# fgiral000/gencast-flax-nnx

Hardware: AMD Instinct MI355X
Metric: denoiser-calls/sec (higher is better)
Workload: dtype f16x3 (every product = 3 fp16 MFMAs on hi/lo-split f32 operands: 22-bit products, f32 accumulate; f32 storage); 1 GPU; nano-GenCast DPM-Solver++2S 20-step sample, 2.5deg grid (73x144), 1 ensemble member per GPU, batch 1; dead_call_skipped=True, grid_nodes=10512, mesh_nodes=2562, latent=256, layers=16, heads=4, ffw_hidden=2048, c_in=262, c_out=82, k_hop=8, parallelism=ensemble-dp1, broadcast=none, rccl_ranks=0, precision=f16x3, library_built_from_this_tree=True, launcher=single

## Files before the change

gencast-flax-nnx_amd/csrc/gc_api.hip:

```cpp
#include <dlfcn.h>

#include "gc_handle.h"

using namespace gci;

namespace {

void protect_pending_noise(gc_handle* h) {
  if (h->guard_pending && h->d_noise == h->last_noise) std::swap(h->d_noise, h->d_noise_alt);
}

int check_ready(gc_handle* h) {
  if (!h) return GC_ERR_INVALID_ARGUMENT;
  if (!h->finalized) return fail(h, GC_ERR_STATE, "gc_finalize has not been called");
  return GC_OK;
}

struct Rccl {
  void* lib = nullptr;
  ncclResult_t (*GetUniqueId)(ncclUniqueId*) = nullptr;
  ncclResult_t (*CommInitRank)(ncclComm_t*, int, ncclUniqueId, int) = nullptr;
  ncclResult_t (*CommDestroy)(ncclComm_t) = nullptr;
  ncclResult_t (*CommCount)(const ncclComm_t, int*) = nullptr;
  ncclResult_t (*CommUserRank)(const ncclComm_t, int*) = nullptr;
// ... 97 lines not shown
  if (hipGetDeviceCount(&n) != hipSuccess) return 0;
  return n;
}

int gc_device_pci_bus_id(int32_t device_id, char* out, int64_t cap) {
  if (!out || cap < 16 || device_id < 0 || device_id >= gc_device_count()) return GC_ERR_INVALID_ARGUMENT;
  out[0] = 0;
  return hipDeviceGetPCIBusId(out, (int)cap, device_id) == hipSuccess ? GC_OK : GC_ERR_HIP;
}

const char* gc_last_error(const gc_handle* h) { return h ? h->err.c_str() : g_create_error.c_str(); }

static void read_switches(gc_handle* h) {
  auto is = [](const char* name, const char* value) { const char* v = std::getenv(name); return v && std::string(v) == value; };
  auto off = [](const char* name) { const char* v = std::getenv(name); return v && *v && std::atoi(v) == 0; };
  auto on = [](const char* name) { const char* v = std::getenv(name); return v && *v == '1'; };
  h->f16x3 = !is("GC_PRECISION", "f32");
  h->use_graphs = !is("GC_TUNE_GRAPH", "0");
  h->m2g_fuse_sum = !off("GC_TUNE_M2G_FUSE_SUM");
  h->embed_cache = !off("GC_TUNE_EMBED_CACHE");
  h->attn_items = !off("GC_TUNE_ATTN_ITEMS");
  h->mlp_pair = !off("GC_TUNE_MLP_PAIR");
  h->edge_terms = !off("GC_TUNE_EDGE_TERMS");
  h->a16 = !off("GC_TUNE_A16");
  h->graph_serialize = on("GC_TUNE_GRAPH_SERIALIZE");
  h->graph_verbose = on("GC_TUNE_GRAPH_VERBOSE");
  h->poison = on("GC_DEBUG_POISON");
}

int gc_create(const gc_config* cfg, int device_id, gc_handle** out) {
  return guarded(nullptr, [&]() -> int {
  if (!cfg || !out) { g_create_error = "null argument"; return GC_ERR_INVALID_ARGUMENT; }
  *out = nullptr;
  const gc_config& c = *cfg;
  auto bad = [&](const char* m) { g_create_error = m; return GC_ERR_INVALID_ARGUMENT; };
  if (c.latent_size <= 0 || c.d_model <= 0 || c.num_heads <= 0 || c.ffw_hidden <= 0 ||
      c.num_layers < 0 || c.c_in <= 0 || c.c_out <= 0 || c.batch <= 0)
    return bad("all dimensions must be positive");
  if (c.c_out > c.c_in) return bad("c_out cannot exceed c_in (noisy targets are part of the forcings)");
  if (c.latent_size != c.d_model) return bad("latent_size must equal d_model");
  if (c.d_model % c.num_heads) return bad("num_heads has to divide d_model exactly");
  if (c.noise_num_frequencies <= 0 || c.noise_num_frequencies > 128 || c.noise_hidden <= 0 ||
      c.noise_hidden > 128 || !(c.noise_base_period > 0))
    return bad("noise encoder sizes out of range");
  auto unsup = [&](const char* m) { g_create_error = m; return GC_ERR_UNSUPPORTED; };
  if (c.latent_size != 128 && c.latent_size != 256 && c.latent_size != 512)
// ... 675 lines not shown
    double n = 1;
    for (auto d : kv.second) n *= (double)d;
    params += n;
  }
  *bytes = 4.0 * (params + G * (c.c_in + c.c_out) + 2 * G * L + NL * M * D * 10);
  *flops = f;
  return GC_OK;
  });
}

int gc_get_counter(gc_handle* h, const char* name, int64_t* value) {
  return guarded(h, [&]() -> int {
  if (!h) return GC_ERR_INVALID_ARGUMENT;
  if (!name || !value) return fail(h, GC_ERR_INVALID_ARGUMENT, "null argument");
  const std::string n(name);
  if (n == "range_fallbacks") *value = h->range_fallbacks;
  else if (n == "static_embedding_fallbacks") *value = h->static_embedding_fallbacks;
  else if (n == "launches_per_call") *value = h->launches_last_call;
  else if (n == "weights_f16_unsafe") *value = h->weights_f16_unsafe ? 1 : 0;
  else if (n == "fp16_storage") *value = h->last_route.st16 ? 1 : 0;
  else if (n == "split_edge") *value = h->split_edge ? 1 : 0;
  else if (n == "attention_items") *value = h->last_route.att_items;
  else if (n == "m2g_fused_sum") *value = h->last_route.m2g_fused ? 1 : 0;
  else if (n == "embed_cache") *value = h->embed_cache_samples;
  else if (n == "edge_term_samples") *value = h->edge_term_samples;
  else if (n == "edge_term_cache_bytes") *value = h->terms.ready ? h->terms.bytes : 0;
  else if (n == "graph_replays") *value = h->graph_replays;
  else if (n == "graph_captures") *value = h->graph_captures;
  else if (n == "loss_evaluations") *value = h->loss_evaluations;
  else if (n == "loss_device_us") *value = h->loss_device_us;
  else if (const int64_t* v = meter_counter(h, n)) *value = *v;
  else if (n == "ens_window_pushes") *value = h->win_pushes;
  else if (n == "ens_window_ring_bytes") {
    const size_t L = h->win_allocs.key[0], M = h->win_allocs.key[1];
    *value = (int64_t)(L * (((M + 1) * h->hg.G * h->cfg.batch * h->cfg.c_out + 3) / 4 * 4) * sizeof(float));
  }
  else if (n == "ens_map_bytes") *value = h->map_set ? h->map_bytes : 0;
  else if (n == "poison_allocs") *value = h->poison_allocs;
  else if (n == "poison_bytes") *value = h->poison_bytes;
  else if (n == "noise_stream") *value = (int64_t)h->nz_stream;
  else if (n == "device_allocations") {
    *value = 0;
    for (const BufferGroup* g : h->groups) *value += (int64_t)g->ptrs.size();
  }
  else return fail(h, GC_ERR_INVALID_ARGUMENT, "unknown counter: " + n);
  return GC_OK;
// ... 499 lines not shown
```

gencast-flax-nnx_amd/csrc/gc_forward.hip:

```cpp
#include "gc_handle.h"

namespace gci {

template <class To, class From>
static const To& a16_view(const From& v) {
  static_assert(sizeof(To) == sizeof(From), "argument struct mismatch between the two kernel builds");
  return reinterpret_cast<const To&>(v);
}

Route make_route(const gc_handle* h) {
  const int D = h->cfg.d_model, F = h->cfg.ffw_hidden;
  Route r;
  r.f16 = h->f16x3 && !h->weights_f16_unsafe && !h->in_fallback;
  r.x32 = !r.f16 && h->f32_ws;
  const bool streams = r.f16 || r.x32;
  r.ffw_slabs = streams ? h->ffw_fused_slabs : 0;
  r.st16 = h->feat16 && h->a16 && r.f16 && D % 128 == 0 && D <= 512 &&
           (h->ffw_fused_slabs > 0 || (F % 128 == 0 && (F / h->ffw2_splits) % 128 == 0));
  r.v2 = r.f16 && r.ws(3 * D, D, 1);
  r.att_items = (h->att_n_items > 0 && r.ws(3 * D, D, 1) && h->attn_splits == 1 && D <= 512) ? h->att_n_items : 0;
  r.fuse_row = streams && D % 128 == 0 && D <= 512;
  r.node_ws = r.f16;
  r.split_edge = h->split_edge;
  r.try_pair = h->mlp_pair && h->hidden_layers == 1;
  r.m2g_fused = h->m2g_fuse_sum && h->hg.m2g_tri && h->hidden_layers == 1 && streams;
  r.embed_cache = h->embed_cache_live && h->embed_cache_ready && !h->feat16 && h->hidden_layers == 1 && streams;
  r.edge_terms = h->embed_cache_live && h->terms.ready && edge_terms_possible(h) && r.f16;
  return r;
}

bool edge_terms_possible(const gc_handle* h) {
  return h->edge_terms && h->f16x3 && !h->weights_f16_unsafe && !h->in_fallback && !h->feat16 && h->hidden_layers == 1 &&
         h->cfg.latent_size == 256 && h->cfg.batch == 1 && h->hg.m2g_tri;
}

static gc::Segment seg(const float* ptr, const int* index, const float* affine, int width, int ld, int bcast) {
  gc::Segment s;
  s.ptr = ptr; s.index = index; s.affine = affine; s.width = width; s.ld = ld; s.bcast = bcast;
  return s;
}

struct MlpCall {
  gc::Segment seg[3] = {};
  gc::AddTerm add[3] = {};
  int nseg = 0, nadd = 0, rows = 0, B = 1, ldo = 0;
  bool ln = true, cond = true;
  const float* residual = nullptr;
// ... 33 lines not shown
  a.cond_stride = h->cond_total;
  a.residual = c.residual; a.out = c.out; a.ldo = c.ldo;
  a.round16 = h->feat16 ? 1 : 0;
  a.round_out = (h->feat16 && c.round_out) ? 1 : 0;
  a.a16 = r.st16 ? 1 : 0;
  a.seg0_f32 = c.seg0_f32 ? 1 : 0;
  a.out_f32 = c.out_f32 ? 1 : 0;
  a.tri = c.tri ? 1 : 0;
  if (c.tri && !gc::mlp_runs_weight_streaming(a))
    return fail(h, GC_ERR_INTERNAL, "the triple-sum epilogue exists in the weight-streaming MLP kernel only");
  return GC_OK;
}

static int enqueue_mlp(gc_handle* h, const gc::MlpArgs& a) {
  return launch(h, gc::KC_MLP, [&] {
    return a.a16 ? gc_a16::launch_mlp(h->stream, a16_view<gc_a16::MlpArgs>(a)) : gc::launch_mlp(h->stream, a);
  });
}
static int enqueue_mlp_pair(gc_handle* h, const gc::MlpArgs& a, const gc::MlpArgs& b) {
  return launch(h, gc::KC_MLP, [&] {
    return a.a16 ? gc_a16::launch_mlp_pair(h->stream, a16_view<gc_a16::MlpArgs>(a), a16_view<gc_a16::MlpArgs>(b))
                 : gc::launch_mlp_pair(h->stream, a, b);
  });
}
static int enqueue_gemm_ws(gc_handle* h, int cls, const gc::GemmArgs& ga, int mt, int splits, int epi) {
  return launch(h, cls, [&] {
    return ga.a16 ? gc_a16::launch_gemm_ws(h->stream, cls, a16_view<gc_a16::GemmArgs>(ga), mt, splits, epi)
                  : gc::launch_gemm_ws(h->stream, cls, ga, mt, splits, epi);
  });
}
static int enqueue_gemm_rowop(gc_handle* h, int cls, const gc::GemmArgs& ga, const gc::RowFuse& rf) {
  return launch(h, cls, [&] {
    return ga.a16 ? gc_a16::launch_gemm_rowop(h->stream, cls, a16_view<gc_a16::GemmArgs>(ga), a16_view<gc_a16::RowFuse>(rf))
                  : gc::launch_gemm_rowop(h->stream, cls, ga, rf);
  });
}
static int enqueue_ffw_fused(gc_handle* h, const gc::FfwArgs& fa) {
  return launch(h, gc::KC_GEMM_FFW1, [&] {
    return fa.a16 ? gc_a16::launch_ffw_fused(h->stream, a16_view<gc_a16::FfwArgs>(fa)) : gc::launch_ffw_fused(h->stream, fa);
  });
}

static int run_mlp_one(gc_handle* h, const DevMlp& w, const MlpCall& c) {
  gc::MlpArgs a{};
  if (int rc = build_mlp_args(h, w, c, &a)) return rc;
  return enqueue_mlp(h, a);
// ... 138 lines not shown
static int mesh_gemm(gc_handle* h, int cls, const float* a, int lda, const Weight& w, int n, int k, int splits,
                     const float* bias, int act, float* out, int ldo, int epi, bool att_merge = false) {
  const Route& r = h->route;
  const bool ws = r.ws(n, k, splits);
  gc::GemmArgs ga = mesh_gemm_args(h, a, lda, ws);
  ga.wt = pick(w, r, ws ? Form::Streaming : Form::Staged); ga.ldw = k; ga.n = n; ga.k_slice = k / splits;
  ga.bias = bias; ga.act = act; ga.out = out; ga.ldo = ldo;
  if (att_merge) merge_attention_partials(h, &ga);
  if (ws) return enqueue_gemm_ws(h, cls, ga, att_merge ? 1 : pick_ws_mt(ga.rows, n, splits), splits, epi);
  return launch(h, cls, [&] { return gc::launch_gemm(h->stream, cls, ga, splits, epi, r.f16); });
}

int forward(gc_handle* h, float sigma_scalar, const float* cond_ready) {
  const gc_config& c = h->cfg;
  const gc::HostGraph& g = h->hg;
  const int B = c.batch, L = c.latent_size, D = c.d_model, F = c.ffw_hidden;
  hipStream_t s = h->stream;
  int rc;
  const float* cond = cond_ready ? cond_ready : h->d_cond;
  h->cond_cur = cond;
  const int cs = h->cond_total;
  const int64_t launches0 = h->launch_count;
  const Route& r = h->route = h->last_route = make_route(h);

  if (!cond_ready && (rc = launch(h, gc::KC_COND, [&] {
         return gc::launch_cond(s, sigma_scalar < 0 ? h->d_sigma : nullptr, sigma_scalar, B, h->d_nw0t,
                                h->d_nb0, h->d_nw1t, h->d_nb1, c.noise_num_frequencies, c.noise_hidden,
                                c.noise_base_period, h->d_wc_all, h->d_bc_all, cs, h->d_condvec,
                                h->d_cond);
       })))
    return rc;

  {
    MlpCall embed = r.embed_cache ? mlp_call({seg(h->d_xn, nullptr, nullptr, h->nwp, h->nwp, 0)}, g.G * B, B, h->d_g0, L)
                                  : mlp_call({seg(h->d_xp, nullptr, nullptr, h->kp, h->kp, 0)}, g.G * B, B, h->d_g0, L);
    embed.seg0_f32 = true;
    if (r.embed_cache) embed.add_terms({{h->d_pstat, nullptr}});
    if ((rc = run_mlp(h, r.embed_cache ? h->g2m_embed_grid_n : h->g2m_embed_grid, embed))) return rc;
  }
  const size_t ML = (size_t)g.M * L;
  if (r.edge_terms && (h->term_slot < 0 || !h->terms.ready))
    return fail(h, GC_ERR_INTERNAL, "edge terms: the forward has no slot of the cache");
  const float* const m0 = r.edge_terms ? h->terms.m0 + h->term_slot * ML : h->d_m0;
  h->m0_cur = m0;
  if (!r.edge_terms && (rc = launch(h, gc::KC_PACK, [&] {
         return gc::launch_affine_rows(s, h->d_m0_hat, cond + h->g2m_embed_mesh.cond_off, cs, g.M, B, L,
// ... 78 lines not shown
    }
    if (stop_here(i, 2)) return GC_OK;
    if (r.ffw_slabs > 0) {
      gc::FfwArgs fa{h->d_h, MB, (int)D, (int)F, pick(ly.w1, r, Form::Streaming), ly.b1, pick(ly.w2, r, Form::Streaming),
                     h->d_part, h->feat16 ? 1 : 0, r.st16 ? 1 : 0};
      fa.f32w = r.x32 ? 1 : 0;
      if ((rc = enqueue_ffw_fused(h, fa))) return rc;
    } else {
      if ((rc = mesh_gemm(h, gc::KC_GEMM_FFW1, h->d_h, D, ly.w1, F, D, 1, ly.b1, 1, h->d_u, F, 0))) return rc;
      if ((rc = mesh_gemm(h, gc::KC_GEMM_FFW2, h->d_u, F, ly.w2, D, F, h->ffw2_splits, nullptr, 0, h->d_part, D, 1))) return rc;
    }
    pend_bias = ly.b2;
    pend_slabs = r.ffw_slabs > 0 ? r.ffw_slabs : h->ffw2_splits;
  }
  if ((rc = rowop(pend_bias, pend_slabs, h->cond_final, h->d_m2))) return rc;

  if ((r.split_edge || r.edge_terms) && (rc = edge_node_products(h, h->m2g_edge, h->d_m2, g.M * B, h->d_pm, h->d_g1, g.G * B, h->d_pg)))
    return rc;
  if ((rc = run_m2g_edge(h, cond, r.m2g_fused))) return rc;
  if (!r.m2g_fused && (rc = launch(h, gc::KC_SEGSUM, [&] {
         return gc::launch_segsum(s, h->d_f1, h->d_m2g_ptr, h->d_m2g_eid, g.G, g.E2, B, L, h->d_agg2, h->feat16, r.st16);
       })))
    return rc;
  if ((rc = run_mlp(h, h->m2g_grid, mlp_call({seg(h->d_g1, nullptr, nullptr, L, L, 0), seg(h->d_agg2, nullptr, nullptr, L, L, 0)},
                                             g.G * B, B, h->d_g2, L, h->d_g1))))
    return rc;
  MlpCall dec = mlp_call({seg(h->d_g2, nullptr, nullptr, L, L, 0)}, g.G * B, B, h->d_y, c.c_out);
  dec.ln = dec.cond = false; dec.out_f32 = true;
  if ((rc = run_mlp(h, h->m2g_dec, dec))) return rc;
  h->launches_last_call = h->launch_count - launches0;
  return GC_OK;
}

int compute_static_embeddings(gc_handle* h) {
  const gc::HostGraph& hg = h->hg;
  const int L = h->cfg.latent_size;
  const struct { const DevMlp& w; const float* in; int items; float* out; } embeds[] = {
      {h->g2m_embed_mesh, h->d_mesh_struct16, hg.M, h->d_m0_hat},
      {h->g2m_embed_edge, h->d_e1_struct16, hg.E1, h->d_e0_hat},
      {h->m2g_embed_edge, h->d_e2_struct16, hg.E2, h->d_f0_hat}};
  if (int rc = drop_edge_terms(h)) return rc;
  auto run = [&]() -> int {
    h->route = make_route(h);
    for (const auto& e : embeds) {
      MlpCall c = mlp_call({seg(e.in, nullptr, nullptr, 32, 32, 1)}, e.items, 1, e.out, L);
      c.cond = c.round_out = false; c.seg0_f32 = c.out_f32 = true;
      if (int rc = run_mlp(h, e.w, c)) return rc;
    }
    return GC_OK;
  };
  if (int rc = run()) return rc;
  GC_HIP(h, hipStreamSynchronize(h->stream));
// ... 91 lines not shown
```

gencast-flax-nnx_amd/csrc/gc_handle.h:

```cpp
#pragma once
#include <hip/hip_runtime.h>

#include <algorithm>
#include <array>
#include <cmath>
#include <cstdio>
#include <cstdlib>
#include <cstring>
#include <map>
#include <memory>
#include <mutex>
#include <string>
#include <type_traits>
#include <vector>

#include <rccl/rccl.h>

#include "../../include/gencast_hip.h"
#include "../../include/gencast_hip_debug.h"
#include "gc_graph.h"
#include "gc_kernels.h"

namespace gci {

inline int round_up(int v, int m) { return (v + m - 1) / m * m; }

struct Route {
  bool f16 = false;
  bool x32 = false;
  bool st16 = false;
  int ffw_slabs = 0;
  bool v2 = false;
  int att_items = 0;
  bool fuse_row = false;
  bool node_ws = false;
  bool m2g_fused = false;
  bool split_edge = false;
  bool try_pair = false;
  bool embed_cache = false;
  bool edge_terms = false;
  bool ws(int n, int k, int splits) const { return (f16 || x32) && n % 128 == 0 && (k / splits) % 128 == 0; }
};

struct Weight {
  float* t = nullptr;
  float* s = nullptr;
  float* f = nullptr;
  float* x = nullptr;
  int ld = 0, kf = 0;
};
enum class Form { Staged, Streaming };
inline const float* pick(const Weight& w, const Route& r, Form form) {
  if (form == Form::Streaming) return r.x32 ? w.x : w.f;
  return r.f16 ? w.s : w.t;
}

struct DevMlp {
  Weight w1, w2;
  Weight w1e, w1snd, w1rcv;
  float *b1 = nullptr, *b2 = nullptr;
  int n_out = 0, n_out_pad = 0;
// ... 142 lines not shown
  int64_t edge_term_cap_mb = 4096;
  EdgeTerms terms;
  gci::BufferGroup term_allocs{groups};
  int term_slot = -1;
  const float* m0_cur = nullptr;
  int64_t edge_term_samples = 0;
  float *d_ones = nullptr, *d_zeros = nullptr;
  int hidden_layers = 1;
  float* d_mlp_tmp[2] = {nullptr, nullptr};
  float *d_feats2 = nullptr, *d_ro_a = nullptr, *d_ro_b = nullptr, *d_ro_forc = nullptr;
  int *d_ro_kind = nullptr, *d_ro_src = nullptr, *d_ro_sidx = nullptr;
  int ro_nforc = -1, ro_forc_cap = 0;
  bool has_sample = false;
  int max_tile_chunks = 0;
  int ffw_fused_slabs = 0;
  void* d_kv16 = nullptr;
  bool f32_ws = true;
  bool split_edge = false;
  int attn_splits = 1, out_splits = 1, ffw2_splits = 1;
  gci::Route route;
  gci::Route last_route;
  bool a16 = true;
  bool attn_items = true;
  bool graph_serialize = false;
  bool graph_verbose = false;
  bool poison = false;
  int64_t poison_allocs = 0, poison_bytes = 0;
  int* d_slots = nullptr;
  float *d_sx = nullptr, *d_sden = nullptr, *d_smid = nullptr, *d_noise = nullptr;
  float *d_noise_alt = nullptr, *last_noise = nullptr;
  float* d_stash = nullptr;
  hipEvent_t ev_stash = nullptr;
  bool has_stash = false;

  int nz_L = 0, nz_lat = 0, nz_lon = 0;
  float *d_nz_leg = nullptr, *d_nz_cos = nullptr, *d_nz_sin = nullptr, *d_nz_coef = nullptr, *d_nz_f = nullptr;
  unsigned long long nz_key = 0, nz_stream = 0;
  std::vector<float> churn_rates;
  float churn_inflation = 1.0f;

  bool has_loss_weights = false, has_targets = false, has_denoised = false;
  int loss_groups = 0;
  float *d_lw_node = nullptr, *d_lw_chan = nullptr, *d_lw_group = nullptr;
  int* d_l_group = nullptr;
  float *d_targets = nullptr, *d_lx = nullptr, *d_lden = nullptr;
  double* d_lpart = nullptr;
// ... 204 lines not shown
  gci::KeyedGroup<3> fss_work_allocs{groups};
  int fss_S = 0;
  int fss_n_lat = 0, fss_n_lon = 0;
  std::vector<int32_t> fss_rlat;
  int *d_fss_rlat = nullptr, *d_fss_rlon = nullptr;
  unsigned* d_fss_roww = nullptr;
  uint2* d_fss_work = nullptr;
  double* d_fss_part = nullptr;
  double* d_fss_out = nullptr;
  gci::Meter fss{events};

  struct SampleGraph {
    std::vector<float> sigmas;
    int skip_dead = 1;
    const float* noise = nullptr;
    bool feat16 = false;
    gci::Route route;
    hipGraph_t graph = nullptr;
    hipGraphExec_t exec = nullptr, exec2 = nullptr;
    hipEvent_t done[2] = {nullptr, nullptr};
    int next = 0;
    int calls = 0;
    int64_t launches_per_call = 0, launches = 0;
    uint64_t last_use = 0;
  };
  bool use_graphs = true;
  std::vector<SampleGraph> sample_graphs;
  uint64_t graph_clock = 0;
  int64_t graph_replays = 0, graph_captures = 0;
  int debug_layer_limit = -1;
  int debug_stop_layer = -1, debug_stop_phase = -1;
  bool f16x3 = true;
  float g2m_agg_norm = 0.f;
  bool feat16 = false;
  bool weights_f16_unsafe = false;
  bool in_fallback = false;
  unsigned* d_nonfinite = nullptr;
  unsigned* h_nonfinite = nullptr;
  unsigned nonfinite_seen = 0;
  int64_t range_fallbacks = 0;
  int64_t static_embedding_fallbacks = 0;
  bool guard_pending = false;
  std::vector<float> last_sigmas;
  int last_skip_dead = 1;
  unsigned long long last_stream0 = 0;
  int64_t launches_last_call = 0, launch_count = 0;
// ... 182 lines not shown
```

gencast-flax-nnx_amd/csrc/gc_kernels.hip:

```cpp
#include "gc_kernels.h"

#include <algorithm>
#include <atomic>
#include <type_traits>

#include <math.h>
#include <stdlib.h>

#ifdef GC_TU_A16
#define GC_TU_NS gc_a16
#else
#define GC_TU_NS gc
#endif
namespace GC_TU_NS {
#ifdef GC_TU_A16
constexpr bool kTuA16 = true;
#else
constexpr bool kTuA16 = false;
#endif

#include "gc_dev_common.inc"


struct DynLdsOnce {
// ... 1032 lines not shown
#pragma unroll
        for (int e = 0; e < 4; ++e)
          if (c + e < n) a.out[(size_t)orow * a.ldo + c + e] = v[e];
      }
    }
  }
  });
}

template <int NT1, int NT2, int MT, int WM, int NWC = 4, int NW2 = NWC,
          int OCC = mlp_ws_occ<NT1, WM, NWC>() , bool A16 = false,
          bool F32 = false, bool TERMS = false>
__global__ __launch_bounds__(64 * NWC * WM, OCC) void gc_mlp_ws_kernel(MlpArgs a) {
  gc_mlp_ws_body<NT1, NT2, MT, WM, NWC, NW2, OCC, A16, F32, TERMS>(a, (int)blockIdx.x);
}

template <int NT1, int NT2, int MT, int WM, int NWC = 4, int NW2 = NWC,
          int OCC = mlp_ws_occ<NT1, WM, NWC>(), bool A16 = false, bool F32 = false, bool TERMS_A = false >
__global__ __launch_bounds__(64 * NWC * WM, OCC) void gc_mlp_ws_pair_kernel(MlpArgs a, MlpArgs b, int na) {
  if ((int)blockIdx.x < na) gc_mlp_ws_body<NT1, NT2, MT, WM, NWC, NW2, OCC, A16, F32, TERMS_A>(a, (int)blockIdx.x);
  else gc_mlp_ws_body<NT1, NT2, MT, WM, NWC, NW2, OCC, A16, F32>(b, (int)blockIdx.x - na);
}

template <int NT1, int NT2, int MT, int WM, int NWC, int NW2>
static hipError_t mlp_ws_geometry(const MlpArgs& a, int* grid_out, size_t* lds_out) {
  constexpr int HID = NT1 * 32 * NWC, NPAD = NT2 * 32 * NW2, BM = 32 * MT * WM;
  constexpr int abuf = 2 * BM * ((BM >= 128 ? 64 : 128) + 4);
  constexpr int region = (abuf > BM * (HID + 4)) ? abuf : BM * (HID + 4);
  static_assert(BM * (NPAD + 4) <= region, "output tile must fit the shared region");
  *lds_out = (size_t)(6 * BM + region) * sizeof(float);
  if (a.nadd < 0 || a.nadd > 3 || (a.nadd > 0 && !a.add[0].ptr) || (a.nadd > 1 && !a.add[1].ptr) || (a.nadd > 2 && !a.add[2].ptr))
    return hipErrorInvalidValue;
  if (a.nseg != 0 && a.nadd > 2) return hipErrorInvalidValue;
  int ksum = 0;
  for (int i = 0; i < a.nseg; ++i) {
    if (a.seg[i].width % 32 || a.seg[i].ld % 4) return hipErrorInvalidValue;
    ksum += a.seg[i].width;
  }
  if (a.nseg == 0) {
    if (a.nadd < 1 || !a.f16 || a.f32w || a.a16 || a.round16 || !a.w2f) return hipErrorInvalidValue;
  } else if (a.k1f % 64 || a.k1f < ksum || a.k1f - ksum >= 64 || !a.w2f || !a.ones || !a.zeros || ksum > 512 * 3) {
    return hipErrorInvalidValue;
  }
  if (kTuA16) {
    constexpr int KCc = BM >= 128 ? 64 : 128;
    for (int i = 0; i < a.nseg; ++i) {
// ... 120 lines not shown
  if (a.f16 || a.a16 || a.tri || !a.w1t || a.nadd < 0 || a.nadd > 2 || a.nseg == 0) return hipErrorInvalidValue;
  for (int i = 0; i < a.nadd; ++i)
    if (!a.add[i].index) return hipErrorInvalidValue;
#define GC_MLP(A_, B_) \
  if (nt1 == A_ && nt2 == B_) return launch_mlp_t<A_, B_, false, 1>(s, a);
  GC_MLP(1, 1) GC_MLP(2, 2) GC_MLP(2, 1) GC_MLP(4, 4) GC_MLP(4, 1)
#undef GC_MLP
  return hipErrorInvalidValue;
}

bool mlp_pair_supported(const MlpArgs& a, const MlpArgs& b) {
  auto ok = [](const MlpArgs& m) {
    if (!mlp_runs_weight_streaming(m) || m.tri || m.n_out_pad != m.hidden) return false;
    return m.hidden == 512 || (m.hidden == 256 && m.rows < kMlpMt2Rows);
  };
  if (b.nseg == 0 || (a.nseg == 0 && a.hidden != 256)) return false;
  return ok(a) && ok(b) && a.hidden == b.hidden && a.f16 == b.f16 && a.f32w == b.f32w && a.a16 == b.a16;
}
hipError_t launch_mlp_pair(hipStream_t s, const MlpArgs& a, const MlpArgs& b) {
  if (!mlp_pair_supported(a, b)) return hipErrorInvalidValue;
  if (a.hidden == 512) return launch_mlp_ws_pair_t<2, 2, 2, 1, 8, 8>(s, a, b);
  if (a.nseg == 0) return launch_mlp_ws_pair_t<1, 1, 1, 1, 8, 8, true>(s, a, b);
  return launch_mlp_ws_pair_t<1, 1, 1, 1, 8, 8>(s, a, b);
}

template <bool H16>
__device__ __forceinline__ f32x4 seg_ld4(const float* base, size_t elem) {
  if constexpr (H16) return ldh4(as_h16(base) + elem);
  else return ld4(base + elem);
}
template <bool H16>
__device__ __forceinline__ void seg_st4(float* base, size_t elem, f32x4 v) {
  if constexpr (H16) sth4(as_h16(base) + elem, v);
  else st4(base + elem, v);
}

template <bool H16>
__global__ __launch_bounds__(256) void gc_segsum_kernel(const float* __restrict__ src,
                                                         const int* __restrict__ rowptr,
                                                         const int* __restrict__ eids, int n_items,
                                                         int B, int width, float* __restrict__ out, int round16,
                                                         float norm ) {
  __shared__ __attribute__((aligned(16))) float part[4][512];
  const int wrow = blockIdx.x;
  const int wave = threadIdx.x >> 6, lane = threadIdx.x & 63;
  const int item = wrow / B, b = wrow - item * B;
// ... 2247 lines not shown
  const size_t total = (size_t)rows * c_out;
  for (size_t i = (size_t)blockIdx.x * 256 + threadIdx.x; i < total; i += (size_t)gridDim.x * 256) {
    const size_t row = i / c_out;
    xp[row * kp + 3 + slots[i - row * c_out]] = 0.f;
  }
}

__global__ __launch_bounds__(256) void gc_scale_kernel(const float* __restrict__ src, float a, size_t n,
                                                        float* __restrict__ dst, NoisyWrite nw) {
  for (size_t i = (size_t)blockIdx.x * 256 + threadIdx.x; i < n; i += (size_t)gridDim.x * 256) {
    const float v = a * src[i];
    dst[i] = v;
    if (nw.xp || nw.xn) put_noisy(nw, i, v);
  }
}

__global__ __launch_bounds__(256) void gc_dpm_first_kernel(const float* __restrict__ y,
                                                            const float* __restrict__ x, float c_out,
                                                            float c_skip, float a_mid, size_t n,
                                                            float* __restrict__ den,
                                                            float* __restrict__ mid, NoisyWrite nw) {
  for (size_t i = (size_t)blockIdx.x * 256 + threadIdx.x; i < n; i += (size_t)gridDim.x * 256) {
    const float xv = x[i];
    const float d = y[i] * c_out + xv * c_skip;
    den[i] = d;
    const float m = a_mid * xv + (1.0f - a_mid) * d;
    mid[i] = m;
    if (nw.xp || nw.xn) put_noisy(nw, i, m);
  }
}

__global__ __launch_bounds__(256) void gc_dpm_second_kernel(const float* __restrict__ y,
                                                             const float* __restrict__ xmid,
                                                             float c_out, float c_skip, float a_next,
                                                             size_t n, float* __restrict__ x, NoisyWrite nw) {
  for (size_t i = (size_t)blockIdx.x * 256 + threadIdx.x; i < n; i += (size_t)gridDim.x * 256) {
    const float md = y[i] * c_out + xmid[i] * c_skip;
    const float v = a_next * x[i] + (1.0f - a_next) * md;
    x[i] = v;
    if (nw.xp || nw.xn) put_noisy(nw, i, v);
  }
}

__global__ __launch_bounds__(256) void gc_affine_rows_kernel(const float* __restrict__ src,
                                                              const float* __restrict__ cond,
                                                              int cond_stride, size_t items, int B,
                                                              int w, float* __restrict__ out, int round16, int h16) {
  const size_t total = items * B * w;
  for (size_t i = (size_t)blockIdx.x * 256 + threadIdx.x; i < total; i += (size_t)gridDim.x * 256) {
    const size_t row = i / w;
    const int c = (int)(i - row * w);
    const size_t item = row / B;
    const int b = (int)(row - item * B);
    const float* cs = cond + (size_t)b * cond_stride;
    const float v = src[item * w + c] * cs[c] + cs[w + c];
    if (h16) as_h16(out)[i] = (_Float16)v;
    else out[i] = r16_if(v, round16);
  }
}

static int ew_grid(size_t n) {
// ... 235 lines not shown
```

gencast-flax-nnx_amd/csrc/gc_kernels_decl.inc:

```
namespace GC_KERNELS_NS {

enum KernelClass : int {
  KC_COND = 0,
  KC_PACK,
  KC_MLP,
  KC_SEGSUM,
  KC_ROWOP,
  KC_GEMM_QKV,
  KC_ATTN,
  KC_ATTN_COMBINE,
  KC_GEMM_OUT,
  KC_GEMM_FFW1,
  KC_GEMM_FFW2,
  KC_GEMM_NODE,
  KC_NOISE,
  KC_COUNT
};

constexpr int kTileM = 32;
constexpr int kCondDim = 16;

struct Segment {
  const float* ptr;
  const int* index;
// ... 155 lines not shown
hipError_t launch_affine_rows(hipStream_t s, const float* src, const float* cond, int cond_stride,
                              int items, int B, int w, float* out, bool round16 = false,
                              bool h16 = false );
hipError_t launch_finite_check(hipStream_t s, const float* p, size_t n, unsigned* counter);
constexpr int kItemPieces = 4;
struct NoisyWrite {
  const int* slots = nullptr;
  int c_out = 1, kp = 0;
  float scale = 0.f;
  float* xp = nullptr;
  float* xn = nullptr;
  int ldn = 0;
  bool active() const { return xp != nullptr || xn != nullptr; }
};
hipError_t launch_scale(hipStream_t s, const float* src, float a, size_t n, float* dst, const NoisyWrite& nw = NoisyWrite());
hipError_t launch_rollout_advance(hipStream_t s, const float* old_feats, const float* sample, const float* forcings,
                                  const int* kind, const int* src, const int* sidx, const float* a, const float* b,
                                  int rows, int c_in, int c_out, int n_forcing, float* new_feats);
hipError_t launch_dpm_first(hipStream_t s, const float* y, const float* x, float c_out, float c_skip,
                            float a_mid, size_t n, float* den, float* mid, const NoisyWrite& nw = NoisyWrite());
hipError_t launch_dpm_second(hipStream_t s, const float* y, const float* xmid, float c_out,
                             float c_skip, float a_next, size_t n, float* x, const NoisyWrite& nw = NoisyWrite());

constexpr int kLossMaxBlocks = 2048;
constexpr int kLossMaxGroups = 64;
constexpr size_t kLossMaxLds = 32 * 1024;
int loss_reduce_blocks(int G, int B, int c_out);
hipError_t launch_loss_noisy(hipStream_t s, const float* t, const float* nz, const float* sigma, const int* slots, int rows,
                             int B, int c_out, int kp, float* x, float* xp);
hipError_t launch_loss_reduce(hipStream_t s, const float* y, const float* t, const float* nz, const float* x,
                              const float* sigma, const float* node_w, int G, int B, int c_out, double* part, float* den);
hipError_t launch_loss_finish(hipStream_t s, const double* part, int blocks, const float* sigma, const float* chan_w,
                              const int* chan_group, const float* group_w, int B, int c_out, int n_groups, float* loss,
                              float* per_group);

hipError_t launch_noise_normals(hipStream_t s, float* out, size_t count, unsigned long long key,
                                unsigned long long stream);
hipError_t launch_noise_synthesis(hipStream_t s, const float* leg, const float* ctab, const float* stab,
                                  const float* coef, float* f, int L, int n_lat, int n_lon, int N,
                                  const float* base, float scale, float* out);

const char* kernel_class_name(int cls);

}
```

gencast-flax-nnx_amd/csrc/gc_sampler.hip:

```cpp
#include "gc_handle.h"

namespace gci {

int guard_enqueue(gc_handle* h, const float* p, size_t n) {
  if (!make_route(h).f16) return GC_OK;
  int rc = launch(h, gc::KC_PACK, [&] { return gc::launch_finite_check(h->stream, p, n, h->d_nonfinite); });
  if (rc) return rc;
  GC_HIP(h, hipMemcpyAsync(h->h_nonfinite, h->d_nonfinite, sizeof(unsigned), hipMemcpyDeviceToHost, h->stream));
  return GC_OK;
}
bool guard_tripped(gc_handle* h) {
  if (*h->h_nonfinite == h->nonfinite_seen) return false;
  h->nonfinite_seen = *h->h_nonfinite;
  return true;
}

float f_c_in(float s) { return 1.0f / std::sqrt(s * s + 1.0f); }
float f_c_out(float s) { return s / std::sqrt(s * s + 1.0f); }
float f_c_skip(float s) { return 1.0f / (s * s + 1.0f); }

int noise_field(gc_handle* h, const float* base, float scale, float* out) {
  if (h->nz_L == 0) return fail(h, GC_ERR_STATE, "gc_noise_set_tables has not been called");
  const int N = h->cfg.batch * h->cfg.c_out;
  const size_t ncoef = (size_t)2 * h->nz_L * h->nz_L * N;
// ... 39 lines not shown
    nw.slots = h->d_slots; nw.c_out = c.c_out; nw.kp = h->kp; nw.scale = f_c_in(std::max(sigma_next_call, 1e-6f));
    if (cache) { nw.xn = h->d_xn; nw.ldn = h->nwp; }
    else nw.xp = h->d_xp;
    return nw;
  };
  auto churned = [&](int i) { return churn && i < n && h->churn_rates[i] > 0.f; };
  bool written = false;
  {
    const gc::NoisyWrite nw = (n > 0 && !churned(0)) ? noisy_write(sigmas[0]) : gc::NoisyWrite();
    if ((rc = launch(h, gc::KC_PACK, [&] { return gc::launch_scale(s, h->d_noise, sigmas[0], ne, h->d_sx, nw); })))
      return rc;
    written = nw.active();
  }
  if (multi) {
    gc::SigmaList sl{};
    for (size_t i = 0; i < call_sigma.size(); ++i) sl.v[i] = call_sigma[i];
    if ((rc = launch(h, gc::KC_COND, [&] {
           return gc::launch_cond_multi(s, sl, (int)call_sigma.size(), c.batch, h->d_nw0t, h->d_nb0, h->d_nw1t,
                                        h->d_nb1, c.noise_num_frequencies, c.noise_hidden, c.noise_base_period,
                                        h->d_wc_all, h->d_bc_all, h->cond_total, h->d_cond_all);
         })))
      return rc;
  }
  auto denoise = [&](const float* x, float sigma) -> int {
    const float ss = std::max(sigma, 1e-6f);
    if (!written) {
      int r = launch(h, gc::KC_PACK, [&] {
        return cache ? gc::launch_write_noisy_compact(s, x, rows, c.c_out, h->nwp, f_c_in(ss), h->d_xn)
                     : gc::launch_write_noisy(s, x, h->d_slots, rows, c.c_out, h->kp, f_c_in(ss), h->d_xp);
      });
      if (r) return r;
    }
    written = false;
    const float* ready = nullptr;
    if (multi) {
      if (calls >= (int)call_sigma.size() || call_sigma[calls] != ss)
        return fail(h, GC_ERR_INTERNAL, "sampler: noise-level list out of step with the loop");
      ready = h->d_cond_all + (size_t)calls * cond_call;
    }
    h->term_slot = route.edge_terms ? h->terms.call_slot[calls] : -1;
    ++calls;
    return forward(h, ss, ready);
  };
  for (int i = 0; i < n; ++i) {
    float sg = sigmas[i];
    const float sn = sigmas[i + 1];
    if (churn && h->churn_rates[i] > 0.f) {
      const float s_new = sg * (1.0f + h->churn_rates[i]);
      const float extra = std::sqrt(std::max(s_new * s_new - sg * sg, 0.0f)) * h->churn_inflation;
      if ((rc = noise_field(h, h->d_sx, extra, h->d_sx))) return rc;
      sg = s_new;
    }
    const float sm = std::sqrt(sg * sn);
    if ((rc = denoise(h->d_sx, sg))) return rc;
    const float ss = std::max(sg, 1e-6f);
    const float a_mid = sm / sg;
    {
      const bool mid_call = (sn != 0.0f) || !skip_dead;
      const gc::NoisyWrite nw = mid_call ? noisy_write(sm) : gc::NoisyWrite();
      if ((rc = launch(h, gc::KC_PACK, [&] {
             return gc::launch_dpm_first(s, h->d_y, h->d_sx, f_c_out(ss), f_c_skip(ss), a_mid, ne,
                                         h->d_sden, h->d_smid, nw);
           })))
        return rc;
      written = nw.active();
    }
    if (sn == 0.0f) {
      if (!skip_dead && (rc = denoise(h->d_smid, sm))) return rc;
      GC_HIP(h, hipMemcpyAsync(h->d_sx, h->d_sden, ne * sizeof(float), hipMemcpyDeviceToDevice, s));
      written = false;
      continue;
    }
    if ((rc = denoise(h->d_smid, sm))) return rc;
    const float sms = std::max(sm, 1e-6f);
    const float a_next = sn / sg;
    {
      const gc::NoisyWrite nw = (i + 1 < n && !churned(i + 1)) ? noisy_write(sigmas[i + 1]) : gc::NoisyWrite();
      if ((rc = launch(h, gc::KC_PACK, [&] {
             return gc::launch_dpm_second(s, h->d_y, h->d_smid, f_c_out(sms), f_c_skip(sms), a_next, ne,
                                          h->d_sx, nw);
           })))
        return rc;
      written = nw.active();
    }
  }
  *calls_out = calls;
  return GC_OK;
}

int run_sampler(gc_handle* h, const float* sigmas, int n, int skip_dead, gc_sample_stats* stats) {
  const gc_config& c = h->cfg;
  const size_t ne = (size_t)h->hg.G * c.batch * c.c_out;
  hipStream_t s = h->stream;
  int rc, calls = 0;
  const unsigned long long stream0 = h->nz_stream;
  const bool churn = !h->churn_rates.empty();
  if (churn && (int)h->churn_rates.size() != n)
    return fail(h, GC_ERR_INVALID_ARGUMENT, "gc_set_churn was given a schedule of another length than this sample");
  std::vector<float> call_sigma;
  for (int i = 0; i < n; ++i) {
    float sg = sigmas[i];
    if (churn && h->churn_rates[i] > 0.f) sg = sg * (1.0f + h->churn_rates[i]);
// ... 34 lines not shown
      sg = nullptr;
    } else {
      sg->last_use = ++h->graph_clock;
    }
  }
  GC_HIP(h, hipEventRecord(h->ev0, s));
  static std::mutex capture_mutex;
  auto launch_exec = [&](gc_handle::SampleGraph* g) -> int {
    std::unique_lock<std::mutex> launch_lock(capture_mutex, std::defer_lock);
    if (h->graph_serialize) launch_lock.lock();
    const int i = g->exec2 ? g->next : 0;
    hipGraphExec_t ex = i ? g->exec2 : g->exec;
    if (!g->done[i]) GC_HIP(h, hipEventCreateWithFlags(&g->done[i], hipEventDisableTiming));
    else GC_HIP(h, hipEventSynchronize(g->done[i]));
    GC_HIP(h, hipGraphLaunch(ex, s));
    GC_HIP(h, hipEventRecord(g->done[i], s));
    g->next = i ^ 1;
    return GC_OK;
  };
  if (sg && sg->exec) {
    if ((rc = launch_exec(sg))) return rc;
    calls = sg->calls;
    h->launches_last_call = sg->launches_per_call;
    h->route = h->last_route = sg->route;
    if (sg->route.edge_terms) ++h->edge_term_samples;
    ++h->graph_replays;
  } else if (sg) {
    const int64_t l0 = h->launch_count;
    auto say = [&](const char* what) { if (h->graph_verbose) { std::fprintf(stderr, "[gc graph] %s\n", what); std::fflush(stderr); } };
    hipGraph_t graph = nullptr;
    hipGraphExec_t exec = nullptr, exec2 = nullptr;
    {
      std::lock_guard<std::mutex> capture_lock(capture_mutex);
      say("begin capture");
      GC_HIP(h, hipStreamBeginCapture(s, hipStreamCaptureModeThreadLocal));
      rc = sampler_body(h, sigmas, n, skip_dead, call_sigma, multi, &calls);
      const hipError_t e_end = hipStreamEndCapture(s, &graph);
      say("end capture");
      if (rc) {
        if (graph) (void)hipGraphDestroy(graph);
        return rc;
      }
      if (e_end != hipSuccess || !graph) return fail(h, GC_ERR_HIP, std::string("hipStreamEndCapture: ") + hipGetErrorString(e_end));
      hipError_t e_inst = hipGraphInstantiate(&exec, graph, nullptr, nullptr, 0);
      if (e_inst == hipSuccess) e_inst = hipGraphInstantiate(&exec2, graph, nullptr, nullptr, 0);
      if (e_inst != hipSuccess) {
        if (exec) (void)hipGraphExecDestroy(exec);
        (void)hipGraphDestroy(graph);
        return fail(h, GC_ERR_HIP, std::string("hipGraphInstantiate: ") + hipGetErrorString(e_inst));
      }
      say("instantiated");
    }
    sg->graph = graph; sg->exec = exec; sg->exec2 = exec2; sg->calls = calls; sg->next = 0;
    sg->launches = h->launch_count - l0;
    sg->launches_per_call = h->launches_last_call;
    sg->route = h->last_route;
    ++h->graph_captures;
    if ((rc = launch_exec(sg))) return rc;
    say("launched");
    ++h->graph_replays;
  } else if ((rc = sampler_body(h, sigmas, n, skip_dead, call_sigma, multi, &calls))) {
    return rc;
  }
  GC_HIP(h, hipEventRecord(h->ev1, s));
  h->has_sample = true;
  if (make_route(h).f16) {
    if ((rc = guard_enqueue(h, h->d_sx, ne))) return rc;
    h->last_sigmas.assign(sigmas, sigmas + n + 1);
    h->last_skip_dead = skip_dead;
    h->guard_pending = true;
    h->last_stream0 = stream0;
    h->last_noise = h->d_noise;
  }
  if (stats) {
    GC_HIP(h, hipEventSynchronize(h->ev1));
    float ms = 0.f;
    GC_HIP(h, hipEventElapsedTime(&ms, h->ev0, h->ev1));
    stats->denoiser_calls = calls;
// ... 72 lines not shown
```

Measured before the change: 762.9 calls/s.

## Chain grid update MLP, decoder MLP and DPM solver step into one kernel

Adds a chained weight-streaming MLP kernel that runs the mesh-to-grid node update MLP and then the decoder MLP on the same row block inside one launch. Optionally it also applies the DPM-Solver++ first or second stage blend on the block's output rows. This removes two kernel launches per denoiser call and the global round trip between the separate kernels, at the cost of a larger fused kernel with its LDS sized to the larger of the two stages. The elementwise DPM formulas now use explicit fmas with contraction disabled, so the fused and unfused paths round the same way.

Result: slower. 691.1 calls/s (-9.4%).

```diff
diff --git a/gencast-flax-nnx_amd/csrc/gc_api.hip b/gencast-flax-nnx_amd/csrc/gc_api.hip
--- a/gencast-flax-nnx_amd/csrc/gc_api.hip
+++ b/gencast-flax-nnx_amd/csrc/gc_api.hip
@@ -143,6 +143,7 @@
   h->attn_items = !off("GC_TUNE_ATTN_ITEMS");
   h->mlp_pair = !off("GC_TUNE_MLP_PAIR");
   h->edge_terms = !off("GC_TUNE_EDGE_TERMS");
+  h->grid_chain = !off("GC_TUNE_GRID_CHAIN");
   h->a16 = !off("GC_TUNE_A16");
   h->graph_serialize = on("GC_TUNE_GRAPH_SERIALIZE");
   h->graph_verbose = on("GC_TUNE_GRAPH_VERBOSE");
@@ -864,6 +865,7 @@
   else if (n == "split_edge") *value = h->split_edge ? 1 : 0;
   else if (n == "attention_items") *value = h->last_route.att_items;
   else if (n == "m2g_fused_sum") *value = h->last_route.m2g_fused ? 1 : 0;
+  else if (n == "grid_chain") *value = h->grid_chain_stages;
   else if (n == "embed_cache") *value = h->embed_cache_samples;
   else if (n == "edge_term_samples") *value = h->edge_term_samples;
   else if (n == "edge_term_cache_bytes") *value = h->terms.ready ? h->terms.bytes : 0;
diff --git a/gencast-flax-nnx_amd/csrc/gc_forward.hip b/gencast-flax-nnx_amd/csrc/gc_forward.hip
--- a/gencast-flax-nnx_amd/csrc/gc_forward.hip
+++ b/gencast-flax-nnx_amd/csrc/gc_forward.hip
@@ -23,6 +23,7 @@
   r.node_ws = r.f16;
   r.split_edge = h->split_edge;
   r.try_pair = h->mlp_pair && h->hidden_layers == 1;
+  r.grid_chain = h->grid_chain && h->hidden_layers == 1 && streams && !h->feat16 && h->cfg.latent_size == 256;
   r.m2g_fused = h->m2g_fuse_sum && h->hg.m2g_tri && h->hidden_layers == 1 && streams;
   r.embed_cache = h->embed_cache_live && h->embed_cache_ready && !h->feat16 && h->hidden_layers == 1 && streams;
   r.edge_terms = h->embed_cache_live && h->terms.ready && edge_terms_possible(h) && r.f16;
@@ -102,6 +103,9 @@
     return a.a16 ? gc_a16::launch_mlp_pair(h->stream, a16_view<gc_a16::MlpArgs>(a), a16_view<gc_a16::MlpArgs>(b))
                  : gc::launch_mlp_pair(h->stream, a, b);
   });
+}
+static int enqueue_mlp_chain(gc_handle* h, const gc::MlpArgs& a, const gc::MlpArgs& b, const gc::ChainTail& t) {
+  return launch(h, gc::KC_MLP, [&] { return gc::launch_mlp_chain(h->stream, a, b, t); });
 }
 static int enqueue_gemm_ws(gc_handle* h, int cls, const gc::GemmArgs& ga, int mt, int splits, int epi) {
   return launch(h, cls, [&] {
@@ -286,6 +290,8 @@
   const int cs = h->cond_total;
   const int64_t launches0 = h->launch_count;
   const Route& r = h->route = h->last_route = make_route(h);
+  h->grid_chain_stages = 0;
+  h->chain_tail_taken = false;
 
   if (!cond_ready && (rc = launch(h, gc::KC_COND, [&] {
          return gc::launch_cond(s, sigma_scalar < 0 ? h->d_sigma : nullptr, sigma_scalar, B, h->d_nw0t,
@@ -410,12 +416,25 @@
          return gc::launch_segsum(s, h->d_f1, h->d_m2g_ptr, h->d_m2g_eid, g.G, g.E2, B, L, h->d_agg2, h->feat16, r.st16);
        })))
     return rc;
-  if ((rc = run_mlp(h, h->m2g_grid, mlp_call({seg(h->d_g1, nullptr, nullptr, L, L, 0), seg(h->d_agg2, nullptr, nullptr, L, L, 0)},
-                                             g.G * B, B, h->d_g2, L, h->d_g1))))
-    return rc;
+  const MlpCall upd = mlp_call({seg(h->d_g1, nullptr, nullptr, L, L, 0), seg(h->d_agg2, nullptr, nullptr, L, L, 0)},
+                               g.G * B, B, h->d_g2, L, h->d_g1);
   MlpCall dec = mlp_call({seg(h->d_g2, nullptr, nullptr, L, L, 0)}, g.G * B, B, h->d_y, c.c_out);
   dec.ln = dec.cond = false; dec.out_f32 = true;
-  if ((rc = run_mlp(h, h->m2g_dec, dec))) return rc;
+  gc::MlpArgs ua{}, da{};
+  bool chained = false;
+  if (r.grid_chain) {
+    if ((rc = build_mlp_args(h, h->m2g_grid, upd, &ua)) || (rc = build_mlp_args(h, h->m2g_dec, dec, &da))) return rc;
+    chained = gc::mlp_chain_supported(ua, da);
+  }
+  if (chained) {
+    const gc::ChainTail tail = h->chain_tail ? *h->chain_tail : gc::ChainTail();
+    if ((rc = enqueue_mlp_chain(h, ua, da, tail))) return rc;
+    h->chain_tail_taken = tail.kind != 0;
+    h->grid_chain_stages = 1 + (tail.kind != 0);
+  } else {
+    if ((rc = run_mlp(h, h->m2g_grid, upd))) return rc;
+    if ((rc = run_mlp(h, h->m2g_dec, dec))) return rc;
+  }
   h->launches_last_call = h->launch_count - launches0;
   return GC_OK;
 }
diff --git a/gencast-flax-nnx_amd/csrc/gc_handle.h b/gencast-flax-nnx_amd/csrc/gc_handle.h
--- a/gencast-flax-nnx_amd/csrc/gc_handle.h
+++ b/gencast-flax-nnx_amd/csrc/gc_handle.h
@@ -37,6 +37,7 @@
   bool m2g_fused = false;
   bool split_edge = false;
   bool try_pair = false;
+  bool grid_chain = false;
   bool embed_cache = false;
   bool edge_terms = false;
   bool ws(int n, int k, int splits) const { return (f16 || x32) && n % 128 == 0 && (k / splits) % 128 == 0; }
@@ -225,6 +226,10 @@
   gci::Route last_route;
   bool a16 = true;
   bool attn_items = true;
+  bool grid_chain = true;
+  const gc::ChainTail* chain_tail = nullptr;
+  bool chain_tail_taken = false;
+  int grid_chain_stages = 0;
   bool graph_serialize = false;
   bool graph_verbose = false;
   bool poison = false;
@@ -475,6 +480,7 @@
     int next = 0;
     int calls = 0;
     int64_t launches_per_call = 0, launches = 0;
+    int grid_chain_stages = 0;
     uint64_t last_use = 0;
   };
   bool use_graphs = true;
diff --git a/gencast-flax-nnx_amd/csrc/gc_kernels.hip b/gencast-flax-nnx_amd/csrc/gc_kernels.hip
--- a/gencast-flax-nnx_amd/csrc/gc_kernels.hip
+++ b/gencast-flax-nnx_amd/csrc/gc_kernels.hip
@@ -1078,6 +1078,50 @@
   else gc_mlp_ws_body<NT1, NT2, MT, WM, NWC, NW2, OCC, A16, F32>(b, (int)blockIdx.x - na);
 }
 
+__device__ __forceinline__ float dpm_blend_first(float yv, float xv, float c_out, float c_skip) {
+#pragma clang fp contract(off)
+  return __builtin_fmaf(xv, c_skip, yv * c_out);
+}
+__device__ __forceinline__ float dpm_blend_second(float yv, float xv, float c_out, float c_skip) {
+#pragma clang fp contract(off)
+  return __builtin_fmaf(yv, c_out, xv * c_skip);
+}
+__device__ __forceinline__ float dpm_mix(float a, float xv, float d) {
+#pragma clang fp contract(off)
+  return __builtin_fmaf(a, xv, (1.0f - a) * d);
+}
+__device__ __forceinline__ void put_noisy(const NoisyWrite& nw, size_t i, float v);
+
+template <int NT1, int NT2, int MT, int WM, int NWC, int NW2A, int NW2B, int OCC, bool F32>
+__global__ __launch_bounds__(64 * NWC * WM, OCC) void gc_mlp_ws_chain_kernel(MlpArgs a, MlpArgs b, ChainTail t) {
+  const int bid = (int)blockIdx.x;
+  gc_mlp_ws_body<NT1, NT2, MT, WM, NWC, NW2A, OCC, false, F32>(a, bid);
+  __threadfence();
+  __syncthreads();
+  gc_mlp_ws_body<NT1, NT2, MT, WM, NWC, NW2B, OCC, false, F32>(b, bid);
+  if (t.kind == 0) return;
+  __threadfence();
+  __syncthreads();
+  constexpr int BM = 32 * MT * WM, NTHR = 64 * NWC * WM;
+  const int r0 = bid * BM, r1 = r0 + BM < b.rows ? r0 + BM : b.rows;
+  const size_t i1 = (size_t)r1 * t.width;
+  for (size_t i = (size_t)r0 * t.width + threadIdx.x; i < i1; i += NTHR) {
+    float v;
+    if (t.kind == 1) {
+      const float xv = t.x[i];
+      const float d = dpm_blend_first(t.y[i], xv, t.c_out, t.c_skip);
+      t.den[i] = d;
+      v = dpm_mix(t.a, xv, d);
+      t.mid[i] = v;
+    } else {
+      const float md = dpm_blend_second(t.y[i], t.x[i], t.c_out, t.c_skip);
+      v = dpm_mix(t.a, t.state[i], md);
+      t.state[i] = v;
+    }
+    if (t.nw.xp || t.nw.xn) put_noisy(t.nw, i, v);
+  }
+}
+
 template <int NT1, int NT2, int MT, int WM, int NWC, int NW2>
 static hipError_t mlp_ws_geometry(const MlpArgs& a, int* grid_out, size_t* lds_out) {
   constexpr int HID = NT1 * 32 * NWC, NPAD = NT2 * 32 * NW2, BM = 32 * MT * WM;
@@ -1244,6 +1288,49 @@
   if (a.hidden == 512) return launch_mlp_ws_pair_t<2, 2, 2, 1, 8, 8>(s, a, b);
   if (a.nseg == 0) return launch_mlp_ws_pair_t<1, 1, 1, 1, 8, 8, true>(s, a, b);
   return launch_mlp_ws_pair_t<1, 1, 1, 1, 8, 8>(s, a, b);
+}
+
+bool mlp_chain_supported(const MlpArgs& a, const MlpArgs& b) {
+  if (kTuA16 || a.a16 || b.a16 || a.round16 || b.round16) return false;
+  auto ok = [](const MlpArgs& m) {
+    return mlp_runs_weight_streaming(m) && !m.tri && m.nseg > 0 && m.hidden == 256 && m.rows < kMlpMt2Rows;
+  };
+  if (!ok(a) || !ok(b) || a.n_out_pad != 256 || b.n_out_pad != 128 || a.rows != b.rows || a.B != b.B || a.f16 != b.f16 || a.f32w != b.f32w) return false;
+  return b.nseg == 1 && b.nadd == 0 && b.seg[0].ptr == a.out && !b.seg[0].index && !b.seg[0].bcast && b.seg[0].ld == a.ldo &&
+         b.seg[0].width == a.n_out && b.residual != a.out;
+}
+static bool chain_tail_ok(const MlpArgs& b, const ChainTail& t) {
+  if (t.kind == 0) return true;
+  if (t.kind != 1 && t.kind != 2) return false;
+  if (t.y != b.out || t.width != b.n_out || b.ldo != b.n_out || !t.x) return false;
+  return t.kind == 1 ? (t.den && t.mid) : (t.state != nullptr);
+}
+template <int NW2B>
+static hipError_t launch_mlp_ws_chain_t(hipStream_t s, const MlpArgs& a, const MlpArgs& b, const ChainTail& t) {
+  if constexpr (kTuA16) return hipErrorInvalidValue;
+  else {
+    int ga = 0, gb = 0;
+    size_t lds_a = 0, lds_b = 0;
+    if (hipError_t e = mlp_ws_geometry<1, 1, 1, 1, 8, 8>(a, &ga, &lds_a)) return e;
+    if (hipError_t e = mlp_ws_geometry<1, 1, 1, 1, 8, NW2B>(b, &gb, &lds_b)) return e;
+    if (ga != gb) return hipErrorInvalidValue;
+    const size_t lds = lds_a > lds_b ? lds_a : lds_b;
+    constexpr int OCC = mlp_ws_occ<1, 1, 8>();
+    if (a.f32w) {
+      static DynLdsOnce once32;
+      if (hipError_t e = once32.ensure((const void*)gc_mlp_ws_chain_kernel<1, 1, 1, 1, 8, 8, NW2B, OCC, true>, (int)lds)) return e;
+      hipLaunchKernelGGL((gc_mlp_ws_chain_kernel<1, 1, 1, 1, 8, 8, NW2B, OCC, true>), dim3(ga), dim3(512), lds, s, a, b, t);
+      return hipGetLastError();
+    }
+    static DynLdsOnce once;
+    if (hipError_t e = once.ensure((const void*)gc_mlp_ws_chain_kernel<1, 1, 1, 1, 8, 8, NW2B, OCC, false>, (int)lds)) return e;
+    hipLaunchKernelGGL((gc_mlp_ws_chain_kernel<1, 1, 1, 1, 8, 8, NW2B, OCC, false>), dim3(ga), dim3(512), lds, s, a, b, t);
+    return hipGetLastError();
+  }
+}
+hipError_t launch_mlp_chain(hipStream_t s, const MlpArgs& a, const MlpArgs& b, const ChainTail& t) {
+  if (!mlp_chain_supported(a, b) || !chain_tail_ok(b, t)) return hipErrorInvalidValue;
+  return launch_mlp_ws_chain_t<4>(s, a, b, t);
 }
 
 template <bool H16>
@@ -3537,9 +3624,9 @@
                                                             float* __restrict__ mid, NoisyWrite nw) {
   for (size_t i = (size_t)blockIdx.x * 256 + threadIdx.x; i < n; i += (size_t)gridDim.x * 256) {
     const float xv = x[i];
-    const float d = y[i] * c_out + xv * c_skip;
+    const float d = dpm_blend_first(y[i], xv, c_out, c_skip);
     den[i] = d;
-    const float m = a_mid * xv + (1.0f - a_mid) * d;
+    const float m = dpm_mix(a_mid, xv, d);
     mid[i] = m;
     if (nw.xp || nw.xn) put_noisy(nw, i, m);
   }
@@ -3550,8 +3637,8 @@
                                                              float c_out, float c_skip, float a_next,
                                                              size_t n, float* __restrict__ x, NoisyWrite nw) {
   for (size_t i = (size_t)blockIdx.x * 256 + threadIdx.x; i < n; i += (size_t)gridDim.x * 256) {
-    const float md = y[i] * c_out + xmid[i] * c_skip;
-    const float v = a_next * x[i] + (1.0f - a_next) * md;
+    const float md = dpm_blend_second(y[i], xmid[i], c_out, c_skip);
+    const float v = dpm_mix(a_next, x[i], md);
     x[i] = v;
     if (nw.xp || nw.xn) put_noisy(nw, i, v);
   }
diff --git a/gencast-flax-nnx_amd/csrc/gc_kernels_decl.inc b/gencast-flax-nnx_amd/csrc/gc_kernels_decl.inc
--- a/gencast-flax-nnx_amd/csrc/gc_kernels_decl.inc
+++ b/gencast-flax-nnx_amd/csrc/gc_kernels_decl.inc
@@ -201,6 +201,20 @@
 hipError_t launch_dpm_second(hipStream_t s, const float* y, const float* xmid, float c_out,
                              float c_skip, float a_next, size_t n, float* x, const NoisyWrite& nw = NoisyWrite());
 
+struct ChainTail {
+  int kind = 0;
+  int width = 0;
+  const float* y = nullptr;
+  const float* x = nullptr;
+  float c_out = 0.f, c_skip = 0.f, a = 0.f;
+  float* den = nullptr;
+  float* mid = nullptr;
+  float* state = nullptr;
+  NoisyWrite nw;
+};
+bool mlp_chain_supported(const MlpArgs& a, const MlpArgs& b);
+hipError_t launch_mlp_chain(hipStream_t s, const MlpArgs& a, const MlpArgs& b, const ChainTail& t = ChainTail());
+
 constexpr int kLossMaxBlocks = 2048;
 constexpr int kLossMaxGroups = 64;
 constexpr size_t kLossMaxLds = 32 * 1024;
diff --git a/gencast-flax-nnx_amd/csrc/gc_sampler.hip b/gencast-flax-nnx_amd/csrc/gc_sampler.hip
--- a/gencast-flax-nnx_amd/csrc/gc_sampler.hip
+++ b/gencast-flax-nnx_amd/csrc/gc_sampler.hip
@@ -85,7 +85,7 @@
          })))
       return rc;
   }
-  auto denoise = [&](const float* x, float sigma) -> int {
+  auto denoise = [&](const float* x, float sigma, const gc::ChainTail* tail = nullptr) -> int {
     const float ss = std::max(sigma, 1e-6f);
     if (!written) {
       int r = launch(h, gc::KC_PACK, [&] {
@@ -103,7 +103,10 @@
     }
     h->term_slot = route.edge_terms ? h->terms.call_slot[calls] : -1;
     ++calls;
-    return forward(h, ss, ready);
+    h->chain_tail = tail;
+    const int r = forward(h, ss, ready);
+    h->chain_tail = nullptr;
+    return r;
   };
   for (int i = 0; i < n; ++i) {
     float sg = sigmas[i];
@@ -115,14 +118,18 @@
       sg = s_new;
     }
     const float sm = std::sqrt(sg * sn);
-    if ((rc = denoise(h->d_sx, sg))) return rc;
     const float ss = std::max(sg, 1e-6f);
     const float a_mid = sm / sg;
     {
       const bool mid_call = (sn != 0.0f) || !skip_dead;
       const gc::NoisyWrite nw = mid_call ? noisy_write(sm) : gc::NoisyWrite();
-      if ((rc = launch(h, gc::KC_PACK, [&] {
-             return gc::launch_dpm_first(s, h->d_y, h->d_sx, f_c_out(ss), f_c_skip(ss), a_mid, ne,
+      gc::ChainTail tail;
+      tail.kind = 1; tail.width = c.c_out; tail.y = h->d_y; tail.x = h->d_sx;
+      tail.c_out = f_c_out(ss); tail.c_skip = f_c_skip(ss); tail.a = a_mid;
+      tail.den = h->d_sden; tail.mid = h->d_smid; tail.nw = nw;
+      if ((rc = denoise(h->d_sx, sg, &tail))) return rc;
+      if (!h->chain_tail_taken && (rc = launch(h, gc::KC_PACK, [&] {
+             return gc::launch_dpm_first(s, h->d_y, h->d_sx, tail.c_out, tail.c_skip, a_mid, ne,
                                          h->d_sden, h->d_smid, nw);
            })))
         return rc;
@@ -134,13 +141,17 @@
       written = false;
       continue;
     }
-    if ((rc = denoise(h->d_smid, sm))) return rc;
     const float sms = std::max(sm, 1e-6f);
     const float a_next = sn / sg;
     {
       const gc::NoisyWrite nw = (i + 1 < n && !churned(i + 1)) ? noisy_write(sigmas[i + 1]) : gc::NoisyWrite();
-      if ((rc = launch(h, gc::KC_PACK, [&] {
-             return gc::launch_dpm_second(s, h->d_y, h->d_smid, f_c_out(sms), f_c_skip(sms), a_next, ne,
+      gc::ChainTail tail;
+      tail.kind = 2; tail.width = c.c_out; tail.y = h->d_y; tail.x = h->d_smid;
+      tail.c_out = f_c_out(sms); tail.c_skip = f_c_skip(sms); tail.a = a_next;
+      tail.state = h->d_sx; tail.nw = nw;
+      if ((rc = denoise(h->d_smid, sm, &tail))) return rc;
+      if (!h->chain_tail_taken && (rc = launch(h, gc::KC_PACK, [&] {
+             return gc::launch_dpm_second(s, h->d_y, h->d_smid, tail.c_out, tail.c_skip, a_next, ne,
                                           h->d_sx, nw);
            })))
         return rc;
@@ -221,6 +232,7 @@
     if ((rc = launch_exec(sg))) return rc;
     calls = sg->calls;
     h->launches_last_call = sg->launches_per_call;
+    h->grid_chain_stages = sg->grid_chain_stages;
     h->route = h->last_route = sg->route;
     if (sg->route.edge_terms) ++h->edge_term_samples;
     ++h->graph_replays;
@@ -253,6 +265,7 @@
     sg->graph = graph; sg->exec = exec; sg->exec2 = exec2; sg->calls = calls; sg->next = 0;
     sg->launches = h->launch_count - l0;
     sg->launches_per_call = h->launches_last_call;
+    sg->grid_chain_stages = h->grid_chain_stages;
     sg->route = h->last_route;
     ++h->graph_captures;
     if ((rc = launch_exec(sg))) return rc;
```
